# myrrix/myrrix-recommender

Measured on AMD Instinct MI355X. Metric: ALS rows solved/sec (full iteration) at k=64, higher is better.
Workload: dtype f32 storage; per-row Gramian: f16x2-split operands (22 bits), f32 accumulate; Cholesky f32

## Files before the change

### myrrix-recommender_amd/csrc/als_kernels.h

```cpp
#pragma once
#include <hip/hip_runtime.h>
#include <stdint.h>

#include <type_traits>

#include "work_plan.h"

namespace mals {

#ifndef MALS_WAVES
#define MALS_WAVES(T, MODE) ((T) <= 4 ? 4 : ((T) == 5 ? 3 : 2))
#endif
#ifndef MALS_WAVES_H
#define MALS_WAVES_H(T, MODE) ((T) <= 2 ? 5 : ((T) <= 4 ? 3 : 2))
#endif

typedef float f32x4 __attribute__((ext_vector_type(4)));
typedef double f64x4 __attribute__((ext_vector_type(4)));

__host__ __device__ constexpr int tri(int T) { return T * (T + 1) / 2; }
__host__ __device__ constexpr int tidx(int T, int i, int j) { return i * T - (i * (i - 1)) / 2 + (j - i); }

constexpr int GRAMIAN_FLUSH_BINADES = 5;
constexpr int YMAX_SLOTS = 64;
// ... 557 lines not shown
    }
    pp.ch = chn;
  }
}

typedef _Float16 f16x8 __attribute__((ext_vector_type(8)));
typedef _Float16 f16x4 __attribute__((ext_vector_type(4)));
typedef _Float16 f16x2 __attribute__((ext_vector_type(2)));
typedef int i32x4 __attribute__((ext_vector_type(4)));
typedef int i32x2 __attribute__((ext_vector_type(2)));

template <int E>
struct ZOp {
  int r[E / 2];
};
template <int E>
__device__ __forceinline__ f32x4 mfma_h(const ZOp<E>& a, const ZOp<E>& b, f32x4 c) {
  if constexpr (E == 8) {
    return __builtin_amdgcn_mfma_f32_16x16x32_f16(__builtin_bit_cast(f16x8, a), __builtin_bit_cast(f16x8, b), c, 0, 0, 0);
  } else {
    return __builtin_amdgcn_mfma_f32_16x16x16f16(__builtin_bit_cast(f16x4, a), __builtin_bit_cast(f16x4, b), c, 0, 0, 0);
  }
}
#ifndef MALS_SPLIT8_MAXT
#define MALS_SPLIT8_MAXT 7
#endif
__host__ __device__ constexpr int split_slots(int T) { return T <= MALS_SPLIT8_MAXT ? 8 : 4; }

__device__ __forceinline__ void chunk_weights_h(const SolveParams& p, Chunk& e, float zscale) {
  chunk_weights(p, e);
  e.w = __builtin_amdgcn_sqrtf(e.w) * zscale;
}

template <int T, int E, bool FULL, int E2>
__device__ __forceinline__ void issue_pair_h(const SolveParams& p, int col_src, int off, int lane, float (&raw)[T][E]) {
  const int c = lane & 15;
  int col[2];
  bperm2_i<8 * E2, 8 * E2 + 4>(off, col_src, col[0], col[1]);
#ifdef MALS_PROFILING
  if (p.flags & 0x400) {
    col[0] &= 0xfff;
    col[1] &= 0xfff;
  }
#endif
#pragma unroll
  for (int i = 0; i < 2; ++i) {
    const int e = 2 * E2 + i;
    const float* ptr = p.M + ((uint64_t)(uint32_t)col[i] * (uint32_t)p.ldm + (uint32_t)c);
#pragma unroll
    for (int v = 0; v < T; ++v) raw[v][e] = ptr[16 * v];
  }
}

template <int E2>
__device__ __forceinline__ void fetch_pair_cols_h(int col_src, int off, int (&col)[2]) {
  bperm2_i_start<8 * E2, 8 * E2 + 4>(off, col_src, col[0], col[1]);
}
template <int T, int E, bool FULL, int E2>
__device__ __forceinline__ void issue_pair_loads_h(const SolveParams& p, int (&col)[2], int lane, float (&raw)[T][E]) {
  const int c = lane & 15;
  bperm2_i_land(col[0], col[1]);
#ifdef MALS_PROFILING
  if (p.flags & 0x400) {
    col[0] &= 0xfff;
    col[1] &= 0xfff;
  }
#endif
#pragma unroll
  for (int i = 0; i < 2; ++i) {
    const int e = 2 * E2 + i;
    const float* ptr = p.M + ((uint64_t)(uint32_t)col[i] * (uint32_t)p.ldm + (uint32_t)c);
#pragma unroll
    for (int v = 0; v < T; ++v) raw[v][e] = ptr[16 * v];
  }
}

template <int T, int E, bool FULL, int PART, int E2, int NTERM = 2>
__device__ __forceinline__ void convert_pair_h(const SolveParams& p, const Chunk& ch, int lane, const float (&raw)[T][E], ZOp<E> (&zh)[T],
                                               ZOp<E> (&zl)[T], float (&bpart)[T], ZOp<E> (&zm)[NTERM == 3 ? T : 1]) {
  constexpr int m0 = E * PART + 2 * E2;
  const float s0 = row_bcast<m0>(ch.w), s1 = row_bcast<m0 + 1>(ch.w);
  const float c0 = row_bcast<m0>(ch.cb), c1 = row_bcast<m0 + 1>(ch.cb);
#pragma unroll
  for (int v = 0; v < T; ++v) {
    const float y0 = raw[v][2 * E2], y1 = raw[v][2 * E2 + 1];
    const float z0 = y0 * s0, z1 = y1 * s1;
    const int hp = pk_rn16(z0, z1);
    const f16x2 hh = __builtin_bit_cast(f16x2, hp);
    zh[v].r[E2] = hp;
    if constexpr (NTERM == 3) {
      const float r0 = fmaf((float)hh[0], -1.f, z0), r1 = fmaf((float)hh[1], -1.f, z1);
      const int mp = pk_rn16(r0, r1);
      const f16x2 mh = __builtin_bit_cast(f16x2, mp);
      zm[v].r[E2] = mp;
      zl[v].r[E2] = pk_rn16(fmaf((float)mh[0], -1.f, r0), fmaf((float)mh[1], -1.f, r1));
    } else {
      zl[v].r[E2] = pk_rn16(fmaf((float)hh[0], -1.f, z0), fmaf((float)hh[1], -1.f, z1));
    }
    bpart[v] = fmaf(c0, y0, bpart[v]);
    bpart[v] = fmaf(c1, y1, bpart[v]);
  }
}

template <int T, int E, bool FULL, int PART, int NTERM = 2>
__device__ __forceinline__ void convert_refill_h(const SolveParams& p, const Chunk& ch, int next_col, int next_off, int lane,
                                                 float (&raw)[T][E], ZOp<E> (&zh)[T], ZOp<E> (&zl)[T], float (&bpart)[T], ZOp<E> (&zm)[NTERM == 3 ? T : 1]) {
#define MALS_SB __builtin_amdgcn_sched_barrier(0)
  int col[2];
  fetch_pair_cols_h<0>(next_col, next_off, col);
  MALS_SB;
  convert_pair_h<T, E, FULL, PART, 0, NTERM>(p, ch, lane, raw, zh, zl, bpart, zm);
  MALS_SB;
  issue_pair_loads_h<T, E, FULL, 0>(p, col, lane, raw);
  fetch_pair_cols_h<1>(next_col, next_off, col);
  MALS_SB;
  convert_pair_h<T, E, FULL, PART, 1, NTERM>(p, ch, lane, raw, zh, zl, bpart, zm);
  MALS_SB;
  issue_pair_loads_h<T, E, FULL, 1>(p, col, lane, raw);
  if constexpr (E == 8) {
    fetch_pair_cols_h<2>(next_col, next_off, col);
    MALS_SB;
    convert_pair_h<T, E, FULL, PART, 2, NTERM>(p, ch, lane, raw, zh, zl, bpart, zm);
    MALS_SB;
    issue_pair_loads_h<T, E, FULL, 2>(p, col, lane, raw);
    fetch_pair_cols_h<3>(next_col, next_off, col);
    MALS_SB;
    convert_pair_h<T, E, FULL, PART, 3, NTERM>(p, ch, lane, raw, zh, zl, bpart, zm);
    MALS_SB;
    issue_pair_loads_h<T, E, FULL, 3>(p, col, lane, raw);
  }
#undef MALS_SB
}

template <int T, int E>
__device__ __forceinline__ void gram_super_step(const ZOp<E> (&zh)[T], const ZOp<E> (&zl)[T], f32x4 (&acc)[tri(T)]) {
#pragma unroll
  for (int i = 0; i < T; ++i)
#pragma unroll
    for (int j = i; j < T; ++j) acc[tidx(T, i, j)] = mfma_h<E>(zh[i], zh[j], acc[tidx(T, i, j)]);
#pragma unroll
  for (int i = 0; i < T; ++i)
#pragma unroll
    for (int j = i; j < T; ++j) acc[tidx(T, i, j)] = mfma_h<E>(zh[i], zl[j], acc[tidx(T, i, j)]);
#pragma unroll
  for (int i = 0; i < T; ++i)
#pragma unroll
    for (int j = i; j < T; ++j) acc[tidx(T, i, j)] = mfma_h<E>(zl[i], zh[j], acc[tidx(T, i, j)]);
}

template <int T, int E>
__device__ __forceinline__ void gram_super_step3(const ZOp<E> (&zh)[T], const ZOp<E> (&zm)[T], const ZOp<E> (&zl)[T], f32x4 (&acc)[tri(T)]) {
#define MALS_GS3(A, B)                                                                                    \
  _Pragma("unroll") for (int i = 0; i < T; ++i) _Pragma("unroll") for (int j = i; j < T; ++j)              \
      acc[tidx(T, i, j)] = mfma_h<E>(A[i], B[j], acc[tidx(T, i, j)])
  MALS_GS3(zl, zh);
  MALS_GS3(zh, zl);
  MALS_GS3(zm, zm);
  MALS_GS3(zm, zh);
  MALS_GS3(zh, zm);
  MALS_GS3(zh, zh);
#undef MALS_GS3
}

template <int T, int E, bool FULL>
__device__ __forceinline__ void prime_row_h(const SolveParams& p, int col_src, int lane, float (&raw)[T][E]) {
  const int rb = (lane & 48) << 2;
  issue_pair_h<T, E, FULL, 0>(p, col_src, rb, lane, raw);
  issue_pair_h<T, E, FULL, 1>(p, col_src, rb, lane, raw);
  if constexpr (E == 8) {
    issue_pair_h<T, E, FULL, 2>(p, col_src, rb, lane, raw);
    issue_pair_h<T, E, FULL, 3>(p, col_src, rb, lane, raw);
  }
}

template <int T, int E, bool FULL, int PART, int NTERM = 2>
__device__ __forceinline__ void super_step_h(const SolveParams& p, const Chunk& ch, const Chunk& chn, int next_col, bool last, int lane,
                                             float (&raw)[T][E], f32x4 (&acc)[tri(T)], float (&bpart)[T]) {
  constexpr int NP = 16 / E;
  const int rb = (lane & 48) << 2;
  ZOp<E> zh[T], zl[T], zm[NTERM == 3 ? T : 1];
  const int same_row_col = PART == NP - 1 ? chn.col : ch.col;
  const int same_row_off = PART == NP - 1 ? rb : rb + 4 * E * (PART + 1);
  convert_refill_h<T, E, FULL, PART, NTERM>(p, ch, last ? next_col : same_row_col, last ? rb : same_row_off, lane, raw, zh, zl, bpart, zm);
  __builtin_amdgcn_sched_barrier(0);
  if constexpr (NTERM == 3) gram_super_step3<T, E>(zh, zm, zl, acc);
  else gram_super_step<T, E>(zh, zl, acc);
  __builtin_amdgcn_sched_barrier(0);
}

template <int T, int E, bool FULL, int NTERM = 2>
__device__ __forceinline__ void gather_row_h(const SolveParams& p, int64_t begin, int len, int lane, float zscale, Chunk& ch,
                                             int next_col, float (&raw)[T][E], f32x4 (&acc)[tri(T)], float (&bpart)[T]) {
  constexpr int NS = 4 * E, NP = 16 / E;
  const int n_ss = (len + NS - 1) / NS;
  for (int q = 0; NP * q < n_ss; ++q) {
    Chunk chn = chunk_issue<true>(p, begin, len, 64 * (q + 1), lane);
    const int ss = NP * q;
    super_step_h<T, E, FULL, 0, NTERM>(p, ch, chn, next_col, ss + 1 >= n_ss, lane, raw, acc, bpart);
    if (ss + 1 < n_ss) {
      if (NP == 2) chunk_weights_h(p, chn, zscale);
      super_step_h<T, E, FULL, 1, NTERM>(p, ch, chn, next_col, ss + 2 >= n_ss, lane, raw, acc, bpart);
    }
    if constexpr (NP == 4) {
      if (ss + 2 < n_ss) super_step_h<T, E, FULL, 2, NTERM>(p, ch, chn, next_col, ss + 3 >= n_ss, lane, raw, acc, bpart);
      if (ss + 3 < n_ss) {
        chunk_weights_h(p, chn, zscale);
        super_step_h<T, E, FULL, 3, NTERM>(p, ch, chn, next_col, ss + 4 >= n_ss, lane, raw, acc, bpart);
      }
    }
    ch = chn;
  }
}

template <int T>
__device__ __forceinline__ void init_acc(const SolveParams& p, f32x4 (&acc)[tri(T)], int lane) {
  if (!(p.flags & 2)) {
    const f32x4* G4 = reinterpret_cast<const f32x4*>(p.Gf) + lane;
#pragma unroll
    for (int t = 0; t < tri(T); ++t) acc[t] = G4[t * 64];
  } else {
#pragma unroll
    for (int t = 0; t < tri(T); ++t) acc[t] = f32x4{0.f, 0.f, 0.f, 0.f};
  }
}

template <int T, bool FULL = false>
__device__ __forceinline__ void add_ridge(const SolveParams& p, f32x4 (&acc)[tri(T)], int n_u, int lane) {
  const int g = lane >> 4, c = lane & 15;
  const float ridge = p.lambda_alpha * (float)n_u;
  float rd[4];
#pragma unroll
  for (int r = 0; r < 4; ++r) rd[r] = (4 * g + r == c) ? ridge : 0.f;
  float w00 = 1.f;
  if constexpr (!FULL) w00 = readlane(acc[tidx(T, 0, 0)][0], 0) + ridge;
#pragma unroll
  for (int v = 0; v < T; ++v) {
    if (FULL || v < T - 1) {
#pragma unroll
      for (int r = 0; r < 4; ++r) acc[tidx(T, v, v)][r] += rd[r];
    } else {
// ... 56 lines not shown
    } else {
#pragma unroll
      for (int r = 0; r < 4; ++r) acc[t][r] *= s2;
    }
  }
#pragma unroll
  for (int v = 0; v < T; ++v) bcol[v] *= s2;
  return inv_s2;
}

template <int T, bool PERM = false>
__device__ __forceinline__ void store_row(const SolveParams& p, float (&xcol)[T], float minpiv, float wmax, int row, int lane) {
  if (!(minpiv > p.sing_threshold)) {
    if (lane == 0) {
      if (p.refine_flag) {
        p.refine_flag[row] = 2;
        *p.any_marked = 1;
      } else {
        atomicMin(p.bad_row, (unsigned long long)row);
      }
    }
#pragma unroll
    for (int v = 0; v < T; ++v) xcol[v] = 0.f;
  } else {
    if (minpiv <= 1024.f * p.sing_threshold && lane == 0) {
      const unsigned long long key = ((unsigned long long)__float_as_uint(minpiv) << 32) | (unsigned)row;
      if (key < __builtin_nontemporal_load(p.suspect)) atomicMin(p.suspect, key);
    }
    if (p.refine_flag && p.refine_limit > 0.f && wmax > p.refine_limit * minpiv && lane == 0) {
      p.refine_flag[row] = 1;
      *p.any_marked = 1;
    }
  }
  if constexpr (PERM) {
    static_assert(T == 8, "the permuted feature order belongs to the k = 128 kernels");
    float* o = p.out + (int64_t)row * p.k;
    int l2 = lane;
    asm volatile("" : "+v"(l2));
    const int g = l2 >> 4, c = l2 & 15;
    const bool hi = ((g ^ (c >> 3)) & 1) != 0;
    f32x4 x;
#pragma unroll
    for (int q = 0; q < 4; ++q) x[q] = hi ? xcol[4 + q] : xcol[q];
    if (g < 2) *reinterpret_cast<f32x4*>(o + 8 * c + 4 * g) = x;
  } else {
    float* o = p.out + (int64_t)row * p.k;
    int l2 = lane;
    asm volatile("" : "+v"(l2));
    const int g = l2 >> 4, c = l2 & 15;
#pragma unroll
    for (int m = 0; 4 * m < T; ++m) {
      const float x = select4(g, xcol[4 * m], 4 * m + 1 < T ? xcol[4 * m + 1] : 0.f, 4 * m + 2 < T ? xcol[4 * m + 2] : 0.f,
                              4 * m + 3 < T ? xcol[4 * m + 3] : 0.f);
      const int feat = 16 * (4 * m + g) + c;
      if (4 * m + 3 < T - 1 || feat < p.k) o[feat] = x;
    }
  }
}

template <int T, bool PERM = false>
__device__ __forceinline__ void finish_row(const SolveParams& p, f32x4 (&acc)[tri(T)], const float (&bcol)[T],
                                           int n_u, int row, int lane, float rmax = 0.f) {
  add_ridge<T, PERM>(p, acc, n_u, lane);
  float minpiv = 3.0e38f;
  float xcol[T];
  const float wmax = fmaxf(rmax, p.gramian_weight * __int_as_float(max_entry_bits<T>(acc, lane)));
  cholesky_tiles<T>(acc, lane, minpiv);
  solve_tiles<T>(acc, bcol, xcol, lane);
// ... 94 lines not shown
          chunk_weights(p, pp.ch);
          prime_row<T, D, FULL>(p, lane, pp);
        }
        solve_tiles<T>(acc, bcol, xcol, lane);
      }
      store_row<T>(p, xcol, minpiv, wmax, cur.id, lane);
#ifdef MALS_PROFILING
      if (tr) {
        t3 = __builtin_readcyclecounter();
        if (lane == 0) {
          unsigned long long* o = p.trace + (trow * 64 + wave) * 6;
          o[0] = t0; o[1] = t1; o[2] = t2; o[3] = t3; o[4] = (unsigned long long)cur.len; o[5] = wall_clock64();
        }
      }
#endif
    } else {
      float* s = p.scratch + (int64_t)cur.id * ((tri(T) * 4 + T) * 64);
#pragma unroll
      for (int t = 0; t < tri(T); ++t) reinterpret_cast<f32x4*>(s)[t * 64 + lane] = acc[t];
#pragma unroll
      for (int v = 0; v < T; ++v) s[(tri(T) * 4 + v) * 64 + lane] = bcol[v];
      if (prime_next) {
        chunk_weights(p, pp.ch);
        prime_row<T, D, FULL>(p, lane, pp);
      }
    }
    if (nxt.len < 0) break;
    cur = nxt;
    nxt = nxt2;
    it += n_waves;
  }
}

template <int T, int MODE, bool FULL, int NTERM = 2>
__global__ __launch_bounds__(256, MALS_WAVES_H(T, MODE)) void als_persistent_kernel_h(SolveParams p) {
  __shared__ f32x4 sG[MODE == 0 ? tri(T) * 64 : 1];
  const int lane = threadIdx.x & 63;
  const int wave = uniform(blockIdx.x * 4 + (threadIdx.x >> 6));
  const int64_t n_waves = (int64_t)gridDim.x * 4;
  if (MODE == 0) {
    const f32x4* G4 = reinterpret_cast<const f32x4*>(p.Gf);
    for (int e = threadIdx.x; e < tri(T) * 64; e += 256) sG[e] = (p.flags & 2) ? f32x4{0.f, 0.f, 0.f, 0.f} : G4[e];
    __syncthreads();
  }
  int64_t it = wave;
  if (it >= p.n_work) return;
  if (p.zscale[2] == 0.f) return;
  const float zscale = __int_as_float(uniform(__float_as_int(p.zscale[0])));
  const float inv_s2 = __int_as_float(uniform(__float_as_int(p.zscale[1])));
  WorkItem cur = load_item(p, it);
  WorkItem nxt = load_item(p, it + n_waves);
  WorkItem nx2 = load_item(p, it + 2 * n_waves);
  constexpr int E = split_slots(T);
  float raw[T][E];
#pragma unroll
  for (int v = 0; v < T; ++v)
#pragma unroll
    for (int e = 0; e < E; ++e) raw[v][e] = 0.f;
  if (cur.len > 0) {
    Chunk ch = chunk_issue<true>(p, cur.begin, cur.len, 0, lane);
    Chunk nch = nxt.len > 0 ? chunk_issue<true>(p, nxt.begin, nxt.len, 0, lane) : ch;
    chunk_weights_h(p, ch, zscale);
    prime_row_h<T, E, FULL>(p, ch.col, lane, raw);
    for (;;) {
      const WorkItem nx3 = load_item(p, it + 3 * n_waves);
      f32x4 acc[tri(T)];
#pragma unroll
      for (int t = 0; t < tri(T); ++t) acc[t] = f32x4{0.f, 0.f, 0.f, 0.f};
      float bpart[T];
#pragma unroll
      for (int v = 0; v < T; ++v) bpart[v] = 0.f;
#ifdef MALS_PROFILING
      const int64_t trow = it / n_waves - p.trace_start;
      const bool tr = MODE == 0 && p.trace && wave < 64 && trow >= 0 && trow < 64;
      unsigned long long t0 = 0, t1 = 0, t2 = 0;
      if (tr) t0 = __builtin_readcyclecounter();
#endif
      gather_row_h<T, E, FULL, NTERM>(p, cur.begin, cur.len, lane, zscale, ch, nch.col, raw, acc, bpart);
#ifdef MALS_PROFILING
      if (tr) t1 = __builtin_readcyclecounter();
#endif
      float bcol[T];
#pragma unroll
      for (int v = 0; v < T; ++v) bcol[v] = reduce_groups(bpart[v], lane);
      ch = nch;
      if (nxt.len > 0) chunk_weights_h(p, ch, zscale);
      if (MODE == 0) {
        const float rmax = p.refine_flag ? __int_as_float(max_entry_bits<T>(acc, lane)) * inv_s2 : 0.f;
#pragma unroll
        for (int t = 0; t < tri(T); ++t) {
          const f32x4 g4 = sG[t * 64 + lane];
          if constexpr (T <= MALS_PK_MAXT) {
            acc[t] = __builtin_elementwise_fma(acc[t], f32x4{inv_s2, inv_s2, inv_s2, inv_s2}, g4);
          } else {
#pragma unroll
            for (int r = 0; r < 4; ++r) acc[t][r] = fmaf(acc[t][r], inv_s2, g4[r]);
          }
        }
        add_ridge<T, FULL>(p, acc, cur.len, lane);
        float minpiv = 3.0e38f, wmax;
        float xcol[T];
        if constexpr (T >= 2) {
          const float inv_s2row = row_scale<T>(acc, bcol, lane, wmax);
          cholesky_tiles<T, true>(acc, lane, minpiv);
          minpiv *= inv_s2row;
        } else {
          wmax = __int_as_float(max_entry_bits<T>(acc, lane));
          cholesky_tiles<T>(acc, lane, minpiv);
        }
#ifdef MALS_PROFILING
        if (tr) t2 = __builtin_readcyclecounter();
#endif
        solve_tiles<T>(acc, bcol, xcol, lane);
        store_row<T>(p, xcol, minpiv, fmaxf(rmax, p.gramian_weight * wmax), cur.id, lane);
#ifdef MALS_PROFILING
        if (tr) {
          const unsigned long long t3 = __builtin_readcyclecounter();
          if (lane == 0) {
            unsigned long long* o = p.trace + (trow * 64 + wave) * 6;
            o[0] = t0; o[1] = t1; o[2] = t2; o[3] = t3; o[4] = (unsigned long long)cur.len; o[5] = wall_clock64();
          }
        }
#endif
      } else {
        float* s = p.scratch + (int64_t)cur.id * ((tri(T) * 4 + T) * 64);
#pragma unroll
        for (int t = 0; t < tri(T); ++t) reinterpret_cast<f32x4*>(s)[t * 64 + lane] = acc[t] * inv_s2;
#pragma unroll
        for (int v = 0; v < T; ++v) s[(tri(T) * 4 + v) * 64 + lane] = bcol[v];
      }
      cur = nxt;
      nxt = nx2;
      nx2 = nx3;
      nch = nxt.len > 0 ? chunk_issue<true>(p, nxt.begin, nxt.len, 0, lane) : nch;
      it += n_waves;
      if (cur.len <= 0) break;
    }
  }
  if (MODE == 0) {
    while (cur.len == 0) {
      f32x4 acc[tri(T)];
#pragma unroll
      for (int t = 0; t < tri(T); ++t) acc[t] = sG[t * 64 + lane];
      float bcol[T];
#pragma unroll
      for (int v = 0; v < T; ++v) bcol[v] = 0.f;
      finish_row<T>(p, acc, bcol, 0, cur.id, lane);
      it += n_waves;
      cur = load_item(p, it);
    }
  }
}

template <int T>
__device__ __forceinline__ void add_slot(const float* __restrict__ s, int lane, f32x4 (&acc)[tri(T)], float (&bcol)[T]) {
  constexpr int PASSES = T >= 6 ? 2 : 1, PER = (tri(T) + PASSES - 1) / PASSES;
#pragma unroll
  for (int ps = 0; ps < PASSES; ++ps) {
    f32x4 part[PER];
#pragma unroll
    for (int t = 0; t < PER; ++t)
      if (ps * PER + t < tri(T)) part[t] = reinterpret_cast<const f32x4*>(s)[(ps * PER + t) * 64 + lane];
    if (ps == 0) {
      float bp[T];
#pragma unroll
      for (int v = 0; v < T; ++v) bp[v] = s[(tri(T) * 4 + v) * 64 + lane];
#pragma unroll
      for (int v = 0; v < T; ++v) bcol[v] += bp[v];
    }
#pragma unroll
    for (int t = 0; t < PER; ++t)
      if (ps * PER + t < tri(T)) acc[ps * PER + t] += part[t];
    if (PASSES > 1) __builtin_amdgcn_sched_barrier(0);
  }
}

template <int T>
__global__ __launch_bounds__(256) void als_prereduce_kernel(SolveParams p) {
  const int lane = threadIdx.x & 63;
  const int64_t wave = (int64_t)blockIdx.x * 4 + (threadIdx.x >> 6);
// ... 824 lines not shown
```

### myrrix-recommender_amd/csrc/lds_kernels.h

```cpp
#pragma once
#include "als_kernels.h"

namespace mals {

constexpr int LDSK_T = 8, LDSK_E = 8;
#ifndef MALS_LDSK_RESPLIT
#define MALS_LDSK_RESPLIT 1
#endif
constexpr bool LDSK_RESPLIT = MALS_LDSK_RESPLIT != 0;
constexpr int LDSK_ROW_BYTES = 512;
constexpr int LDSK_RING_BYTES = 32 * LDSK_ROW_BYTES;
constexpr int LDSK_CHUNK_BYTES = 512;
constexpr int LDSK_NCHUNK = 3;
constexpr int LDSK_WAVE_BYTES = LDSK_RING_BYTES + LDSK_NCHUNK * LDSK_CHUNK_BYTES;

__host__ __device__ constexpr int ldsk_feature(int v, int c) { return 8 * c + (v ^ (4 * (c >> 3))); }

typedef __attribute__((address_space(3))) char lds_char;

__device__ __forceinline__ void glds16(const void* a, unsigned dst) {
  unsigned keep;
  asm volatile(
      "s_mov_b32 %0, m0\n\t"
      "s_mov_b32 m0, %2\n\ts_nop 0\n\tglobal_load_lds_dwordx4 %1, off\n\t"
// ... 77 lines not shown

template <int E2>
__device__ __forceinline__ void ldsk_pair(const lds_char* lds, unsigned ring, float w, float cb, unsigned next_cols, const LdskLane& L,
                                          ZOp<LDSK_E> (&zh)[LDSK_T], ZOp<LDSK_E> (&zl)[LDSK_T], float (&bpart)[LDSK_T]) {
  wait_vm<12>();
  const float s0 = row_bcast<2 * E2>(w), s1 = row_bcast<2 * E2 + 1>(w);
  const float c0 = row_bcast<2 * E2>(cb), c1 = row_bcast<2 * E2 + 1>(cb);
  {
    const f32x4 ya = *reinterpret_cast<lds_f4>(lds + L.rd0 + 4096 * E2);
    const f32x4 yb = *reinterpret_cast<lds_f4>(lds + L.rd0 + 4096 * E2 + 512);
    ldsk_convert_half<E2, 0>(ya, yb, s0, s1, c0, c1, zh, zl, bpart);
  }
  __builtin_amdgcn_sched_barrier(0);
  {
    const f32x4 ya = *reinterpret_cast<lds_f4>(lds + (L.rd0 ^ 16u) + 4096 * E2);
    const f32x4 yb = *reinterpret_cast<lds_f4>(lds + (L.rd0 ^ 16u) + 4096 * E2 + 512);
    ldsk_convert_half<E2, 4>(ya, yb, s0, s1, c0, c1, zh, zl, bpart);
  }
  __builtin_amdgcn_sched_barrier(0);
  ldsk_issue_pair<E2>(lds, ring, next_cols, L);
  __builtin_amdgcn_sched_barrier(0);
}
__device__ __forceinline__ void ldsk_super_step(const lds_char* lds, unsigned ring, float w, float cb, unsigned next_cols, const LdskLane& L,
                                                f32x4 (&acc)[tri(LDSK_T)], float (&bpart)[LDSK_T]) {
  ZOp<LDSK_E> zh[LDSK_T], zl[LDSK_T];
  ldsk_pair<0>(lds, ring, w, cb, next_cols, L, zh, zl, bpart);
  ldsk_pair<1>(lds, ring, w, cb, next_cols, L, zh, zl, bpart);
  ldsk_pair<2>(lds, ring, w, cb, next_cols, L, zh, zl, bpart);
  ldsk_pair<3>(lds, ring, w, cb, next_cols, L, zh, zl, bpart);
  gram_super_step<LDSK_T, LDSK_E>(zh, zl, acc);
  __builtin_amdgcn_sched_barrier(0);
}

__global__ void gramian_perm_kernel(const double* __restrict__ G, int k, float* __restrict__ Gp) {
  constexpr int T = LDSK_T;
  const int e = blockIdx.x * blockDim.x + threadIdx.x;
  if (e >= tri(T) * 256) return;
  const int t = e >> 8, lane = (e >> 2) & 63, reg = e & 3;
  int i = 0, rem = t;
  while (rem >= T - i) {
    rem -= T - i;
    ++i;
  }
  const int j = i + rem;
  const int row = ldsk_feature(i, 4 * (lane >> 4) + reg), col = ldsk_feature(j, lane & 15);
  Gp[e] = (row < k && col < k) ? (float)G[(int64_t)row * k + col] : 0.f;
}

template <int MODE>
__global__ __launch_bounds__(64, 2) void als_lds_kernel_h(SolveParams p) {
  constexpr int T = LDSK_T;
  __shared__ __attribute__((aligned(1024))) char lds_raw[LDSK_WAVE_BYTES];
  const lds_char* lds = (const lds_char*)lds_raw;
  const unsigned lbase = (unsigned)(uintptr_t)lds;
  const int lane = threadIdx.x;
  const int64_t wave = blockIdx.x, n_waves = gridDim.x;
  int64_t it = wave;
  if (it >= p.n_work) return;
  if (p.zscale[2] == 0.f) return;
  const float zscale = __int_as_float(uniform(__float_as_int(p.zscale[0])));
  const float inv_s2 = __int_as_float(uniform(__float_as_int(p.zscale[1])));
  LdskLane L;
  {
    const int g = lane >> 4, c = lane & 15;
    L.rd0 = (unsigned)(g * 1024 + 32 * c + 16 * (c >> 3));
    L.gsrc = reinterpret_cast<const char*>(p.M) + 16 * (lane & 31);
  }
  const unsigned ring = lbase;
  unsigned b_cur = LDSK_RING_BYTES, b_next = LDSK_RING_BYTES + LDSK_CHUNK_BYTES, b_nrow = LDSK_RING_BYTES + 2 * LDSK_CHUNK_BYTES;
  const f32x4* Gp4 = reinterpret_cast<const f32x4*>(p.Gperm);
  WorkItem cur = load_item(p, it);
  WorkItem nxt = load_item(p, it + n_waves);
  WorkItem nx2 = load_item(p, it + 2 * n_waves);
  if (cur.len > 0) {
    ldsk_chunk_dma(p, cur.begin, cur.len, 0, lbase + b_cur, lane);
    if (nxt.len > 0) ldsk_chunk_dma(p, nxt.begin, nxt.len, 0, lbase + b_nrow, lane);
    wait_vm<0>();
    {
// ... 121 lines not shown
```

### myrrix-recommender_amd/csrc/mals_api.hip

```cpp
#include "../../include/myrrix_als.h"
#include "als_kernels.h"
#include "dual_kernels.h"
#include "lds_kernels.h"
#include "host_eigen.h"
#include "host_solver.h"
#include "mals_internal.h"
#include "mals_handle.h"
#include "hip_buffer.h"
#include "work_plan.h"

#include <hip/hip_runtime.h>

#include <algorithm>
#include <chrono>
#include <cmath>
#include <cstdio>
#include <cstdlib>
#include <cstring>
#include <limits>
#include <new>
#include <string>
#include <type_traits>
#include <vector>

// ... 372 lines not shown
    if (!r.n) continue;
    p.n_work = r.n;
    p.items = r.items;
    if (int rc = r.kind ? launch_persistent(h, fam.segments, fam.segments_f32, fam.block, fam.resident_per_cu, p, 1, r.bytes, r.front)
                        : launch_persistent(h, fam.rows, fam.rows_f32, fam.block, fam.resident_per_cu, p, 0, r.bytes, r.front))
      return rc;
  }
  if (longs && cr.nC) {
    PendingEvent pe;
    if (int rc = begin_timed(h, 2, (double)cr.nC * per, pe)) return rc;
    if (cr.nP) {
      p.n_work = cr.nP;
      p.rowsC = s.rowsC.get() + cr.offP;
      hipLaunchKernelGGL(fam.prereduce, dim3((unsigned)((cr.nP + 3) / 4)), dim3(256), 0, h->stream, p);
    }
    p.n_work = cr.nC;
    p.rowsC = s.rowsC.get() + cr.offC;
    hipLaunchKernelGGL(fam.finish, dim3((unsigned)((cr.nC + 3) / 4)), dim3(256), 0, h->stream, p);
    if constexpr (!std::is_same<decltype(fam.finish_f32), std::nullptr_t>::value) {
      SolveParams pf = p;
      pf.flags |= 8;
      hipLaunchKernelGGL(fam.finish_f32, dim3((unsigned)((cr.nC + 3) / 4)), dim3(256), 0, h->stream, pf);
    }
    if (int rc = end_timed(h, pe)) return rc;
  }
  if (own && cr.nZ) {
    hipLaunchKernelGGL(zero_rows_kernel, dim3((unsigned)((cr.nZ + 31) / 32)), dim3(256), 0, h->stream,
                       A + cr.nA + n_dual, cr.nZ, p.k, p.out);
  }
  HIPCHK(h, hipGetLastError());
  return MALS_OK;
}

template <int T, bool FULL>
int launch_solve_TF(mals_handle h, SideState& s, const SolveParams& p, int chunk, int which) {
  constexpr int D = gather_depth(T);
  constexpr auto rows_f32 = als_persistent_kernel<T, D, 0, FULL>;
  constexpr auto segments_f32 = als_persistent_kernel<T, D, 1, FULL>;
  if constexpr (T == 8 && FULL) {
    if (h->split_f16 && h->lds_gather && p.Gperm)
      return launch_lists(h, s, p, chunk, which, ListKernels{als_lds_kernel_h<0>, als_lds_kernel_h<1>, rows_f32, segments_f32, als_finish_kernel<T, true>,
                                                             als_finish_kernel<T, false>, als_prereduce_kernel<T>, 64, 8});
  }
  if constexpr (T == 4) {
    if (h->split3)
      return launch_lists(h, s, p, chunk, which, ListKernels{als_persistent_kernel_h<T, 0, FULL, 3>, als_persistent_kernel_h<T, 1, FULL, 3>, rows_f32,
                                                             segments_f32, als_finish_kernel<T>, nullptr, als_prereduce_kernel<T>, 256, 0});
  }
  if (h->split_f16)
    return launch_lists(h, s, p, chunk, which, ListKernels{als_persistent_kernel_h<T, 0, FULL>, als_persistent_kernel_h<T, 1, FULL>, rows_f32,
                                                           segments_f32, als_finish_kernel<T>, nullptr, als_prereduce_kernel<T>, 256, 0});
  return launch_lists(h, s, p, chunk, which,
                      ListKernels{rows_f32, segments_f32, nullptr, nullptr, als_finish_kernel<T>, nullptr, als_prereduce_kernel<T>, 256, 0});
}

int launch_solve(mals_handle h, SideState& s, const SolveParams& p, int chunk, int which) {
  return dispatch_T(h, [&](auto t) {
    return p.k == 16 * t() ? launch_solve_TF<t(), true>(h, s, p, chunk, which) : launch_solve_TF<t(), false>(h, s, p, chunk, which);
  });
}

int launch_refine(mals_handle h, const RefineParams& q) {
  const int64_t rows = q.row_end - q.row_begin;
  const unsigned grid = (unsigned)std::max<int64_t>(1, std::min<int64_t>((rows + 255) / 256, (int64_t)h->n_cu * 8));
  return dispatch_T(h, [&](auto t) -> int {
    hipLaunchKernelGGL((als_refine_kernel<t()>), dim3(grid), dim3(256), 0, h->stream, q);
    HIPCHK(h, hipGetLastError());
    return MALS_OK;
  });
}

int launch_gramian_ref(mals_handle h, const SideState& o) {
  const unsigned grid = (unsigned)std::max<int64_t>(1, std::min<int64_t>((o.n_total + 63) / 64, (int64_t)h->n_cu * 2));
  return dispatch_T(h, [&](auto t) -> int {
    hipLaunchKernelGGL(gramian_ref_latch_kernel, dim3(1), dim3(1), 0, h->stream, h->d_gref_state.get());
// ... 425 lines not shown
  }
  if (h->cfg.flags != 0 || !(cfg->alpha > 0.0)) h->dual_blocks = 0;
  {
    hipDeviceProp_t prop;
    if (hipGetDeviceProperties(&prop, cfg->device) == hipSuccess && prop.multiProcessorCount > 0)
      h->n_cu = prop.multiProcessorCount;
  }
  std::memset(&h->stats, 0, sizeof(h->stats));
  h->stats.struct_size = (int32_t)sizeof(mals_stats);
  hipError_t st = hipSetDevice(cfg->device);
  if (st == hipSuccess) st = h->d_bad.alloc(4);
  if (st == hipSuccess) st = h->h_bad.alloc(4);
  if (st == hipSuccess) st = h->d_zscale.alloc(4);
  if (st == hipSuccess) st = h->d_maxabs.alloc(4);
  if (st == hipSuccess) st = h->d_colrange.alloc(2);
  if (st == hipSuccess) st = h->d_refined.alloc(1);
  if (st == hipSuccess) st = h->d_gref_state.alloc(4);
  if (st == hipSuccess) st = hipMemset(h->d_gref_state.get(), 0, 4 * sizeof(int));
  if (st == hipSuccess) st = hipMemset(h->d_refined.get(), 0, sizeof(unsigned long long));
  if (st == hipSuccess) st = hipMemset(h->d_zscale.get(), 0, 4 * sizeof(float));
  if (st == hipSuccess) st = hipMemset(h->d_bad.get(), 0xff, 4 * sizeof(unsigned long long));
  if (st != hipSuccess) {
    delete h;
    return create_fail(MALS_HIP_ERROR, "mals_create: device " + std::to_string(cfg->device) + ": " + hipGetErrorString(st));
  }
  if (const char* e = std::getenv("MALS_REFINE_LIMIT")) h->refine_limit = std::max(0.f, (float)std::atof(e));
  if (hipEventCreateWithFlags(&h->ev_ready, hipEventDisableTiming) != hipSuccess ||
      hipEventCreateWithFlags(&h->ev_refine, hipEventDisableTiming) != hipSuccess) {
    delete h;
    return create_fail(MALS_HIP_ERROR, "mals_create: hipEventCreate failed");
  }
  h->lds_gather = h->cfg.features == 128;
  if (const char* e = std::getenv("MALS_LDS_GATHER")) h->lds_gather = h->lds_gather && std::atoi(e) != 0;
  if (const char* e = std::getenv("MALS_OVERLAP")) h->overlap = std::atoi(e) != 0;
  if (h->overlap) {
    bool ok = hipEventCreateWithFlags(&h->ev_fork, hipEventDisableTiming) == hipSuccess;
    for (int i = 0; i < 2 && ok; ++i)
      ok = hipStreamCreateWithFlags(&h->aux[i], hipStreamNonBlocking) == hipSuccess &&
           hipEventCreateWithFlags(&h->ev_join[i], hipEventDisableTiming) == hipSuccess;
    if (!ok) h->overlap = false;
  }
#ifdef MALS_PROFILING
  if (std::getenv("MALS_DEBUG_TRACE")) {
    (void)h->d_trace.alloc(64 * 64 * 6);
    (void)hipMemset(h->d_trace.get(), 0, 64 * 64 * 6 * sizeof(unsigned long long));
  }
#endif
  t_create_error.clear();
  malsi_serving_create(h);
  *out = h;
  return MALS_OK;
}

int mals_destroy(mals_handle h) {
  if (!h) return MALS_INVALID_ARG;
  (void)hipSetDevice(h->cfg.device);
  malsi_serving_stop_front(h);
  (void)hipStreamSynchronize(h->stream);
  if (h->d_trace) {
    std::vector<unsigned long long> t(64 * 64 * 6);
    (void)hipMemcpy(t.data(), h->d_trace.get(), t.size() * sizeof(unsigned long long), hipMemcpyDeviceToHost);
    for (int r = 0; r < 64; r += 21)
      for (int w = 0; w < 4; w += 1) {
        const unsigned long long* o = &t[(size_t)(r * 64 + w) * 6];
        std::fprintf(stderr, "[trace] iter %2d wave %2d len %5llu gather %7llu chol %7llu solve+store %7llu gap_to_prev_end %lld\n", r, w, o[4],
                     o[1] - o[0], o[2] - o[1], o[3] - o[2], r ? (long long)(o[0] - t[(size_t)((r - 1) * 64 + w) * 6 + 3]) : 0ll);
// ... 398 lines not shown
static int solve_setup(mals_handle h, int side, int chunk_begin, int chunk_end, bool g_to_host) {
  SideState& s = h->side[side];
  SideState& o = h->side[1 - side];
  const int k = h->cfg.features;
  const HalfStamp now{side, o.G_version};
  bool new_half = h->pad != now || h->pad_epoch != o.F_epoch || h->pad_done.size() != s.chunks.size();
  for (int c = chunk_begin; c < chunk_end && !new_half; ++c) new_half = h->pad_done[(size_t)c] != 0;
  if (new_half) {
    h->pad = now;
    h->pad_epoch = o.F_epoch;
    h->pad_done.assign(s.chunks.size(), 0);
    h->tl[0] = now_us();
    h->tl[1] = h->tl[2] = 0.0;
    HIPCHK(h, hipMemsetAsync(h->d_gref_state.get(), 0, 3 * sizeof(int), h->stream));
  }
  for (int c = chunk_begin; c < chunk_end; ++c) h->pad_done[(size_t)c] = 1;
  if (k % 16 != 0) {
    const int ld = 16 * h->T;
    const size_t need = (size_t)o.n_total * (size_t)ld;
    if (need > h->d_Mp.capacity()) {
      new_half = true;
      HIPCHK(h, h->d_Mp.reserve(need, h->stream));
    }
    if (new_half) {
      PendingEvent pe;
      if (int rc = begin_timed(h, 5, (double)o.n_total * 4.0 * (k + ld), pe)) return rc;
      const int64_t n4 = o.n_total * (ld / 4);
      const unsigned blocks = (unsigned)std::min<int64_t>((n4 + 255) / 256, (int64_t)h->n_cu * 32);
      hipLaunchKernelGGL(pad_rows_kernel, dim3(blocks ? blocks : 1), dim3(256), 0, h->stream, o.F, o.n_total, k, ld, h->d_Mp.get());
      HIPCHK(h, hipGetLastError());
      if (int rc = end_timed(h, pe)) return rc;
    }
  }
  if (h->lds_gather && h->split_f16 && k == 128) {
    if (!h->d_Gperm) HIPCHK(h, h->d_Gperm.alloc((size_t)tri(8) * 256));
    if (h->gperm != now) {
      if (h->cfg.flags & MALS_FLAG_LOSS_IGNORES_UNSPECIFIED) {
        HIPCHK(h, hipMemsetAsync(h->d_Gperm.get(), 0, sizeof(float) * (size_t)tri(8) * 256, h->stream));
      } else {
        hipLaunchKernelGGL(gramian_perm_kernel, dim3((unsigned)tri(8)), dim3(256), 0, h->stream, o.G.get(), k, h->d_Gperm.get());
        HIPCHK(h, hipGetLastError());
      }
      h->gperm = now;
    }
  }
  HIPCHK(h, s.refine.reserve((size_t)s.n_local, h->stream));
  if (h->split_f16 && (h->zs != now || h->zs_bound != s.max_abs_val || h->zs_mean != s.mean_abs_val)) {
    const double base_w = (h->cfg.flags & MALS_FLAG_LOSS_IGNORES_UNSPECIFIED) ? 1.0 : 0.0;
    const double w_max = base_w + ((h->cfg.flags & MALS_FLAG_RECONSTRUCT_R) ? 0.0 : std::fabs(h->cfg.alpha) * (double)s.max_abs_val);
    const double w_mean = base_w + ((h->cfg.flags & MALS_FLAG_RECONSTRUCT_R) ? 0.0 : std::fabs(h->cfg.alpha) * s.mean_abs_val);
    int force = -1;
    if (const char* e = std::getenv("MALS_FORCE_RANGE_FLAG")) force = std::atoi(e) != 0;
    hipLaunchKernelGGL(gather_scale_kernel, dim3(1), dim3(64), 0, h->stream, o.G.get(), k, (float)std::sqrt(w_max), (float)std::sqrt(w_mean),
                       (double)o.n_total, force, (o.ymax_version != 0 && o.ymax_version == o.G_version) ? o.d_ymax.get() : nullptr, h->d_zscale.get());
    HIPCHK(h, hipGetLastError());
    h->zs = now;
    h->zs_bound = s.max_abs_val;
    h->zs_mean = s.mean_abs_val;
  }
  if (g_to_host) {
    if (!h->h_G) HIPCHK(h, h->h_G.alloc((size_t)k * k));
    if (!h->ev_G) HIPCHK(h, hipEventCreateWithFlags(&h->ev_G, hipEventDisableTiming));
    HIPCHK(h, hipMemcpyAsync(h->h_G.get(), o.G.get(), sizeof(double) * (size_t)k * k, hipMemcpyDeviceToHost, h->stream));
    HIPCHK(h, hipEventRecord(h->ev_G, h->stream));
  }
  return MALS_OK;
}

static SolveParams solve_params(mals_handle h, int side) {
  SideState& s = h->side[side];
  SideState& o = h->side[1 - side];
  const int k = h->cfg.features;
  SolveParams p;
  p.row_ptr = s.row_ptr;
  p.col = s.col;
  p.val = s.val;
  p.M = o.F;
  p.ldm = k;
  if (k % 16 != 0) {
    p.M = h->d_Mp.get();
    p.ldm = 16 * h->T;
  }
  p.Gf = o.Gf.get();
  p.Gperm = h->lds_gather && h->split_f16 && k == 128 ? h->d_Gperm.get() : nullptr;
  p.out = s.F + s.row_offset * k;
  p.items = nullptr;
  p.rowsC = s.rowsC.get();
  p.scratch = s.scratch.get();
  p.bad_row = h->d_bad.get() + side;
  p.suspect = h->d_bad.get() + 2 + side;
  p.any_marked = h->d_gref_state.get();
  p.refine_flag = s.refine.get();
  p.refine_limit = (h->cfg.flags & MALS_FLAG_LOSS_IGNORES_UNSPECIFIED) ? h->refine_limit / 16.f : h->refine_limit;
  p.gramian_weight = 0.25f;
  if (h->cfg.flags & MALS_FLAG_RECONSTRUCT_R) {
    p.gramian_weight = 1.f;
    p.refine_limit *= 0.25f;
  }
  p.n_work = 0;
  p.trace = h->d_trace.get();
  p.trace_start = 0;
  if (const char* ts = std::getenv("MALS_DEBUG_TRACE")) p.trace_start = std::atoi(ts);
  if (const char* ts = std::getenv("MALS_DEBUG_TRACE_SIDE")) if (std::atoi(ts) != side) p.trace = nullptr;
  p.k = k;
  p.flags = h->cfg.flags;
  p.alpha = (float)h->cfg.alpha;
  p.lambda_alpha = (float)(h->cfg.lambda * h->cfg.alpha);
  p.sing_threshold = (float)h->cfg.singularity_threshold;
  p.zscale = h->d_zscale.get();
  return p;
}

static int solve_one_chunk(mals_handle h, int side, const SolveParams& p, int c, int phase, bool want_dual, bool prepare_dual, bool* dual_now) {
  SideState& s = h->side[side];
  const SideState& o = h->side[1 - side];
  const ChunkRange& cr = s.chunks[(size_t)c];
  const bool resume = phase == SOLVE_END;
// ... 520 lines not shown
```

### myrrix-recommender_amd/csrc/mals_handle.h

```cpp
#pragma once
#include "../../include/myrrix_als.h"
#include "hip_buffer.h"
#include "host_solver.h"
#include "work_plan.h"

#include <hip/hip_runtime.h>

#include <atomic>
#include <cstdint>
#include <string>
#include <vector>

struct ServingState;

namespace mals __attribute__((visibility("hidden"))) {

struct SideState {
  int64_t n_total = 0;
  float* F = nullptr;
  DeviceBuffer<float> F_own;
  int64_t row_offset = 0, n_local = 0, nnz = 0;
  int64_t* row_ptr = nullptr;
  int32_t* col = nullptr;
  float* val = nullptr;
// ... 73 lines not shown
  float refine_limit = 64.f;
  bool exact_ready = false;
  DeviceBuffer<int> d_gref_state;
  DeviceBuffer<double> d_Gref;
  DeviceBuffer<double> d_gref_part;
  DeviceBuffer<unsigned long long> d_refined;
  HalfStamp pad;
  uint64_t pad_epoch = 0;
  std::vector<uint8_t> pad_done;
  DeviceBuffer<char> d_eig;
  double* d_Q = nullptr;
  float* d_Qf = nullptr;
  bool rotate_f64 = false;
  bool rotate_split = false;
  int32_t* d_Bs = nullptr;
  size_t Bs_stride = 0;
  float* d_lam = nullptr;
  DeviceBuffer<unsigned> d_zbound;
  PinnedBuffer<double> h_G;
  hipEvent_t ev_G = nullptr;
  PinnedBuffer<char> eig_stage;
  bool eig_ok = false;
  double eig_gmax = 0.0;
  bool dual_pending = false;
  int dual_pending_side = -1, dual_pending_chunk = -1;
  double tl[4] = {0.0, 0.0, 0.0, 0.0};
  HalfStamp dual;
  bool dual_ok = false;
  hipEvent_t ev_ready = nullptr, ev_refine = nullptr;
  bool refine_recorded = false;
  mals_iteration_fn iter_fn = nullptr;
  void* iter_user = nullptr;
  bool lds_gather = false;
  DeviceBuffer<float> d_Gperm;
  HalfStamp gperm;
  DeviceBuffer<float> d_zscale;
  HalfStamp zs;
  float zs_bound = -1.f;
  double zs_mean = -1.0;
  DeviceBuffer<unsigned> d_maxabs;
  DeviceBuffer<int> d_colrange;
  int n_cu = 256;
  SideState side[2];
  hipStream_t stream = nullptr;
  hipStream_t aux[2] = {nullptr, nullptr};
  hipEvent_t ev_fork = nullptr, ev_join[2] = {nullptr, nullptr};
  bool overlap = false;
  bool forked[2] = {false, false};
  std::string err;
  DeviceBuffer<unsigned long long> d_bad;
  PinnedBuffer<unsigned long long> h_bad;
  int32_t sing_side = -1;
  int64_t sing_row = -1;
  int32_t sing_rank = 0;
  std::atomic<int> cancelled{0};
  bool timing = false;
  mals_stats stats;
  std::vector<PendingEvent> pending;
  DeviceBuffer<unsigned long long> d_trace;
  ServingState* serving = nullptr;
  DeviceBuffer<uint32_t> tag_bits;
  int64_t tag_bits_items = 0, n_tag_items = 0;
  const int64_t* known_ptr = nullptr;
  const int32_t* known_idx = nullptr;
  int64_t known_rows = 0;
  DeviceBuffer<int64_t> known_ptr_copy;
// ... 75 lines not shown
```

Before: 139.0 million.

## Use permuted feature order for k=64 so each lane gathers one 16-byte vector

For k=64 row solves, lane c now owns features 4c..4c+3, so each gathered factor row entry is fetched with a single 16-byte vector load instead of four strided scalar loads. The prior Gramian is permuted to match on the device, and the solved row is written back with a 16-byte store from 16 lanes. This cuts gather instruction count and should improve coalescing on the memory-bound gather. The cost is an extra Gperm buffer and permute kernel whenever the Gramian changes, plus more kernel instantiations.

```diff
diff --git a/myrrix-recommender_amd/csrc/als_kernels.h b/myrrix-recommender_amd/csrc/als_kernels.h
--- a/myrrix-recommender_amd/csrc/als_kernels.h
+++ b/myrrix-recommender_amd/csrc/als_kernels.h
@@ -613,7 +613,27 @@
   e.w = __builtin_amdgcn_sqrtf(e.w) * zscale;
 }
 
-template <int T, int E, bool FULL, int E2>
+__host__ __device__ constexpr int perm4_feature(int v, int c) { return 4 * c + v; }
+template <int T, int E, bool FULL, bool PERM>
+__device__ __forceinline__ void load_entry_h(const SolveParams& p, int col, int c, int e, float (&raw)[T][E]) {
+#ifdef MALS_GATHER16_ABLATION
+  constexpr bool X4 = T == 4 && E == 8 && FULL;
+#else
+  constexpr bool X4 = PERM;
+#endif
+  if constexpr (X4) {
+    static_assert(T == 4 && FULL, "the 16-byte gather belongs to k = 64");
+    const f32x4 q = *reinterpret_cast<const f32x4*>(p.M + ((uint64_t)(uint32_t)col * (uint32_t)p.ldm + (uint32_t)(4 * c)));
+#pragma unroll
+    for (int v = 0; v < T; ++v) raw[v][e] = q[v];
+  } else {
+    const float* ptr = p.M + ((uint64_t)(uint32_t)col * (uint32_t)p.ldm + (uint32_t)c);
+#pragma unroll
+    for (int v = 0; v < T; ++v) raw[v][e] = ptr[16 * v];
+  }
+}
+
+template <int T, int E, bool FULL, int E2, bool PERM = false>
 __device__ __forceinline__ void issue_pair_h(const SolveParams& p, int col_src, int off, int lane, float (&raw)[T][E]) {
   const int c = lane & 15;
   int col[2];
@@ -627,9 +647,7 @@
 #pragma unroll
   for (int i = 0; i < 2; ++i) {
     const int e = 2 * E2 + i;
-    const float* ptr = p.M + ((uint64_t)(uint32_t)col[i] * (uint32_t)p.ldm + (uint32_t)c);
-#pragma unroll
-    for (int v = 0; v < T; ++v) raw[v][e] = ptr[16 * v];
+    load_entry_h<T, E, FULL, PERM>(p, col[i], c, e, raw);
   }
 }
 
@@ -637,7 +655,7 @@
 __device__ __forceinline__ void fetch_pair_cols_h(int col_src, int off, int (&col)[2]) {
   bperm2_i_start<8 * E2, 8 * E2 + 4>(off, col_src, col[0], col[1]);
 }
-template <int T, int E, bool FULL, int E2>
+template <int T, int E, bool FULL, int E2, bool PERM = false>
 __device__ __forceinline__ void issue_pair_loads_h(const SolveParams& p, int (&col)[2], int lane, float (&raw)[T][E]) {
   const int c = lane & 15;
   bperm2_i_land(col[0], col[1]);
@@ -650,9 +668,7 @@
 #pragma unroll
   for (int i = 0; i < 2; ++i) {
     const int e = 2 * E2 + i;
-    const float* ptr = p.M + ((uint64_t)(uint32_t)col[i] * (uint32_t)p.ldm + (uint32_t)c);
-#pragma unroll
-    for (int v = 0; v < T; ++v) raw[v][e] = ptr[16 * v];
+    load_entry_h<T, E, FULL, PERM>(p, col[i], c, e, raw);
   }
 }
 
@@ -683,7 +699,7 @@
   }
 }
 
-template <int T, int E, bool FULL, int PART, int NTERM = 2>
+template <int T, int E, bool FULL, int PART, int NTERM = 2, bool PERM = false>
 __device__ __forceinline__ void convert_refill_h(const SolveParams& p, const Chunk& ch, int next_col, int next_off, int lane,
                                                  float (&raw)[T][E], ZOp<E> (&zh)[T], ZOp<E> (&zl)[T], float (&bpart)[T], ZOp<E> (&zm)[NTERM == 3 ? T : 1]) {
 #define MALS_SB __builtin_amdgcn_sched_barrier(0)
@@ -692,23 +708,23 @@
   MALS_SB;
   convert_pair_h<T, E, FULL, PART, 0, NTERM>(p, ch, lane, raw, zh, zl, bpart, zm);
   MALS_SB;
-  issue_pair_loads_h<T, E, FULL, 0>(p, col, lane, raw);
+  issue_pair_loads_h<T, E, FULL, 0, PERM>(p, col, lane, raw);
   fetch_pair_cols_h<1>(next_col, next_off, col);
   MALS_SB;
   convert_pair_h<T, E, FULL, PART, 1, NTERM>(p, ch, lane, raw, zh, zl, bpart, zm);
   MALS_SB;
-  issue_pair_loads_h<T, E, FULL, 1>(p, col, lane, raw);
+  issue_pair_loads_h<T, E, FULL, 1, PERM>(p, col, lane, raw);
   if constexpr (E == 8) {
     fetch_pair_cols_h<2>(next_col, next_off, col);
     MALS_SB;
     convert_pair_h<T, E, FULL, PART, 2, NTERM>(p, ch, lane, raw, zh, zl, bpart, zm);
     MALS_SB;
-    issue_pair_loads_h<T, E, FULL, 2>(p, col, lane, raw);
+    issue_pair_loads_h<T, E, FULL, 2, PERM>(p, col, lane, raw);
     fetch_pair_cols_h<3>(next_col, next_off, col);
     MALS_SB;
     convert_pair_h<T, E, FULL, PART, 3, NTERM>(p, ch, lane, raw, zh, zl, bpart, zm);
     MALS_SB;
-    issue_pair_loads_h<T, E, FULL, 3>(p, col, lane, raw);
+    issue_pair_loads_h<T, E, FULL, 3, PERM>(p, col, lane, raw);
   }
 #undef MALS_SB
 }
@@ -743,18 +759,18 @@
 #undef MALS_GS3
 }
 
-template <int T, int E, bool FULL>
+template <int T, int E, bool FULL, bool PERM = false>
 __device__ __forceinline__ void prime_row_h(const SolveParams& p, int col_src, int lane, float (&raw)[T][E]) {
   const int rb = (lane & 48) << 2;
-  issue_pair_h<T, E, FULL, 0>(p, col_src, rb, lane, raw);
-  issue_pair_h<T, E, FULL, 1>(p, col_src, rb, lane, raw);
+  issue_pair_h<T, E, FULL, 0, PERM>(p, col_src, rb, lane, raw);
+  issue_pair_h<T, E, FULL, 1, PERM>(p, col_src, rb, lane, raw);
   if constexpr (E == 8) {
-    issue_pair_h<T, E, FULL, 2>(p, col_src, rb, lane, raw);
-    issue_pair_h<T, E, FULL, 3>(p, col_src, rb, lane, raw);
-  }
-}
-
-template <int T, int E, bool FULL, int PART, int NTERM = 2>
+    issue_pair_h<T, E, FULL, 2, PERM>(p, col_src, rb, lane, raw);
+    issue_pair_h<T, E, FULL, 3, PERM>(p, col_src, rb, lane, raw);
+  }
+}
+
+template <int T, int E, bool FULL, int PART, int NTERM = 2, bool PERM = false>
 __device__ __forceinline__ void super_step_h(const SolveParams& p, const Chunk& ch, const Chunk& chn, int next_col, bool last, int lane,
                                              float (&raw)[T][E], f32x4 (&acc)[tri(T)], float (&bpart)[T]) {
   constexpr int NP = 16 / E;
@@ -762,14 +778,14 @@
   ZOp<E> zh[T], zl[T], zm[NTERM == 3 ? T : 1];
   const int same_row_col = PART == NP - 1 ? chn.col : ch.col;
   const int same_row_off = PART == NP - 1 ? rb : rb + 4 * E * (PART + 1);
-  convert_refill_h<T, E, FULL, PART, NTERM>(p, ch, last ? next_col : same_row_col, last ? rb : same_row_off, lane, raw, zh, zl, bpart, zm);
+  convert_refill_h<T, E, FULL, PART, NTERM, PERM>(p, ch, last ? next_col : same_row_col, last ? rb : same_row_off, lane, raw, zh, zl, bpart, zm);
   __builtin_amdgcn_sched_barrier(0);
   if constexpr (NTERM == 3) gram_super_step3<T, E>(zh, zm, zl, acc);
   else gram_super_step<T, E>(zh, zl, acc);
   __builtin_amdgcn_sched_barrier(0);
 }
 
-template <int T, int E, bool FULL, int NTERM = 2>
+template <int T, int E, bool FULL, int NTERM = 2, bool PERM = false>
 __device__ __forceinline__ void gather_row_h(const SolveParams& p, int64_t begin, int len, int lane, float zscale, Chunk& ch,
                                              int next_col, float (&raw)[T][E], f32x4 (&acc)[tri(T)], float (&bpart)[T]) {
   constexpr int NS = 4 * E, NP = 16 / E;
@@ -777,16 +793,16 @@
   for (int q = 0; NP * q < n_ss; ++q) {
     Chunk chn = chunk_issue<true>(p, begin, len, 64 * (q + 1), lane);
     const int ss = NP * q;
-    super_step_h<T, E, FULL, 0, NTERM>(p, ch, chn, next_col, ss + 1 >= n_ss, lane, raw, acc, bpart);
+    super_step_h<T, E, FULL, 0, NTERM, PERM>(p, ch, chn, next_col, ss + 1 >= n_ss, lane, raw, acc, bpart);
     if (ss + 1 < n_ss) {
       if (NP == 2) chunk_weights_h(p, chn, zscale);
-      super_step_h<T, E, FULL, 1, NTERM>(p, ch, chn, next_col, ss + 2 >= n_ss, lane, raw, acc, bpart);
+      super_step_h<T, E, FULL, 1, NTERM, PERM>(p, ch, chn, next_col, ss + 2 >= n_ss, lane, raw, acc, bpart);
     }
     if constexpr (NP == 4) {
-      if (ss + 2 < n_ss) super_step_h<T, E, FULL, 2, NTERM>(p, ch, chn, next_col, ss + 3 >= n_ss, lane, raw, acc, bpart);
+      if (ss + 2 < n_ss) super_step_h<T, E, FULL, 2, NTERM, PERM>(p, ch, chn, next_col, ss + 3 >= n_ss, lane, raw, acc, bpart);
       if (ss + 3 < n_ss) {
         chunk_weights_h(p, chn, zscale);
-        super_step_h<T, E, FULL, 3, NTERM>(p, ch, chn, next_col, ss + 4 >= n_ss, lane, raw, acc, bpart);
+        super_step_h<T, E, FULL, 3, NTERM, PERM>(p, ch, chn, next_col, ss + 4 >= n_ss, lane, raw, acc, bpart);
       }
     }
     ch = chn;
@@ -909,8 +925,13 @@
       *p.any_marked = 1;
     }
   }
-  if constexpr (PERM) {
-    static_assert(T == 8, "the permuted feature order belongs to the k = 128 kernels");
+  if constexpr (PERM && T == 4) {
+    float* o = p.out + (int64_t)row * p.k;
+    int l2 = lane;
+    asm volatile("" : "+v"(l2));
+    if (l2 < 16) *reinterpret_cast<f32x4*>(o + 4 * l2) = f32x4{xcol[0], xcol[1], xcol[2], xcol[3]};
+  } else if constexpr (PERM) {
+    static_assert(T == 8, "the permuted feature orders belong to the k = 64 and k = 128 kernels");
     float* o = p.out + (int64_t)row * p.k;
     int l2 = lane;
     asm volatile("" : "+v"(l2));
@@ -1071,14 +1092,15 @@
   }
 }
 
-template <int T, int MODE, bool FULL, int NTERM = 2>
+template <int T, int MODE, bool FULL, int NTERM = 2, bool PERM = false>
 __global__ __launch_bounds__(256, MALS_WAVES_H(T, MODE)) void als_persistent_kernel_h(SolveParams p) {
+  static_assert(!PERM || (T == 4 && FULL && MODE == 0), "the permuted feature order is the k = 64 rows kernel's");
   __shared__ f32x4 sG[MODE == 0 ? tri(T) * 64 : 1];
   const int lane = threadIdx.x & 63;
   const int wave = uniform(blockIdx.x * 4 + (threadIdx.x >> 6));
   const int64_t n_waves = (int64_t)gridDim.x * 4;
   if (MODE == 0) {
-    const f32x4* G4 = reinterpret_cast<const f32x4*>(p.Gf);
+    const f32x4* G4 = reinterpret_cast<const f32x4*>(PERM ? p.Gperm : p.Gf);
     for (int e = threadIdx.x; e < tri(T) * 64; e += 256) sG[e] = (p.flags & 2) ? f32x4{0.f, 0.f, 0.f, 0.f} : G4[e];
     __syncthreads();
   }
@@ -1100,7 +1122,7 @@
     Chunk ch = chunk_issue<true>(p, cur.begin, cur.len, 0, lane);
     Chunk nch = nxt.len > 0 ? chunk_issue<true>(p, nxt.begin, nxt.len, 0, lane) : ch;
     chunk_weights_h(p, ch, zscale);
-    prime_row_h<T, E, FULL>(p, ch.col, lane, raw);
+    prime_row_h<T, E, FULL, PERM>(p, ch.col, lane, raw);
     for (;;) {
       const WorkItem nx3 = load_item(p, it + 3 * n_waves);
       f32x4 acc[tri(T)];
@@ -1115,7 +1137,7 @@
       unsigned long long t0 = 0, t1 = 0, t2 = 0;
       if (tr) t0 = __builtin_readcyclecounter();
 #endif
-      gather_row_h<T, E, FULL, NTERM>(p, cur.begin, cur.len, lane, zscale, ch, nch.col, raw, acc, bpart);
+      gather_row_h<T, E, FULL, NTERM, PERM>(p, cur.begin, cur.len, lane, zscale, ch, nch.col, raw, acc, bpart);
 #ifdef MALS_PROFILING
       if (tr) t1 = __builtin_readcyclecounter();
 #endif
@@ -1151,7 +1173,7 @@
         if (tr) t2 = __builtin_readcyclecounter();
 #endif
         solve_tiles<T>(acc, bcol, xcol, lane);
-        store_row<T>(p, xcol, minpiv, fmaxf(rmax, p.gramian_weight * wmax), cur.id, lane);
+        store_row<T, PERM>(p, xcol, minpiv, fmaxf(rmax, p.gramian_weight * wmax), cur.id, lane);
 #ifdef MALS_PROFILING
         if (tr) {
           const unsigned long long t3 = __builtin_readcyclecounter();
@@ -1184,7 +1206,7 @@
       float bcol[T];
 #pragma unroll
       for (int v = 0; v < T; ++v) bcol[v] = 0.f;
-      finish_row<T>(p, acc, bcol, 0, cur.id, lane);
+      finish_row<T, PERM>(p, acc, bcol, 0, cur.id, lane);
       it += n_waves;
       cur = load_item(p, it);
     }
diff --git a/myrrix-recommender_amd/csrc/lds_kernels.h b/myrrix-recommender_amd/csrc/lds_kernels.h
--- a/myrrix-recommender_amd/csrc/lds_kernels.h
+++ b/myrrix-recommender_amd/csrc/lds_kernels.h
@@ -133,8 +133,7 @@
   __builtin_amdgcn_sched_barrier(0);
 }
 
-__global__ void gramian_perm_kernel(const double* __restrict__ G, int k, float* __restrict__ Gp) {
-  constexpr int T = LDSK_T;
+__global__ void gramian_perm_kernel(const double* __restrict__ G, int k, int T, float* __restrict__ Gp) {
   const int e = blockIdx.x * blockDim.x + threadIdx.x;
   if (e >= tri(T) * 256) return;
   const int t = e >> 8, lane = (e >> 2) & 63, reg = e & 3;
@@ -144,7 +143,8 @@
     ++i;
   }
   const int j = i + rem;
-  const int row = ldsk_feature(i, 4 * (lane >> 4) + reg), col = ldsk_feature(j, lane & 15);
+  const int rc = 4 * (lane >> 4) + reg, cc = lane & 15;
+  const int row = T == LDSK_T ? ldsk_feature(i, rc) : perm4_feature(i, rc), col = T == LDSK_T ? ldsk_feature(j, cc) : perm4_feature(j, cc);
   Gp[e] = (row < k && col < k) ? (float)G[(int64_t)row * k + col] : 0.f;
 }
 
diff --git a/myrrix-recommender_amd/csrc/mals_api.hip b/myrrix-recommender_amd/csrc/mals_api.hip
--- a/myrrix-recommender_amd/csrc/mals_api.hip
+++ b/myrrix-recommender_amd/csrc/mals_api.hip
@@ -428,6 +428,10 @@
   return MALS_OK;
 }
 
+static bool uses_gperm(mals_handle h) {
+  return h->split_f16 && ((h->lds_gather && h->cfg.features == 128) || (h->gather16 && h->cfg.features == 64));
+}
+
 template <int T, bool FULL>
 int launch_solve_TF(mals_handle h, SideState& s, const SolveParams& p, int chunk, int which) {
   constexpr int D = gather_depth(T);
@@ -437,6 +441,15 @@
     if (h->split_f16 && h->lds_gather && p.Gperm)
       return launch_lists(h, s, p, chunk, which, ListKernels{als_lds_kernel_h<0>, als_lds_kernel_h<1>, rows_f32, segments_f32, als_finish_kernel<T, true>,
                                                              als_finish_kernel<T, false>, als_prereduce_kernel<T>, 64, 8});
+  }
+  if constexpr (T == 4 && FULL) {
+    if (h->split_f16 && h->gather16 && p.Gperm) {
+      if (h->split3)
+        return launch_lists(h, s, p, chunk, which, ListKernels{als_persistent_kernel_h<T, 0, FULL, 3, true>, als_persistent_kernel_h<T, 1, FULL, 3>, rows_f32,
+                                                               segments_f32, als_finish_kernel<T>, nullptr, als_prereduce_kernel<T>, 256, 0});
+      return launch_lists(h, s, p, chunk, which, ListKernels{als_persistent_kernel_h<T, 0, FULL, 2, true>, als_persistent_kernel_h<T, 1, FULL>, rows_f32,
+                                                             segments_f32, als_finish_kernel<T>, nullptr, als_prereduce_kernel<T>, 256, 0});
+    }
   }
   if constexpr (T == 4) {
     if (h->split3)
@@ -928,6 +941,8 @@
   }
   h->lds_gather = h->cfg.features == 128;
   if (const char* e = std::getenv("MALS_LDS_GATHER")) h->lds_gather = h->lds_gather && std::atoi(e) != 0;
+  h->gather16 = h->cfg.features == 64;
+  if (const char* e = std::getenv("MALS_K64_GATHER16")) h->gather16 = h->gather16 && std::atoi(e) != 0;
   if (const char* e = std::getenv("MALS_OVERLAP")) h->overlap = std::atoi(e) != 0;
   if (h->overlap) {
     bool ok = hipEventCreateWithFlags(&h->ev_fork, hipEventDisableTiming) == hipSuccess;
@@ -1392,13 +1407,13 @@
       if (int rc = end_timed(h, pe)) return rc;
     }
   }
-  if (h->lds_gather && h->split_f16 && k == 128) {
-    if (!h->d_Gperm) HIPCHK(h, h->d_Gperm.alloc((size_t)tri(8) * 256));
+  if (uses_gperm(h)) {
+    if (!h->d_Gperm) HIPCHK(h, h->d_Gperm.alloc((size_t)tri(h->T) * 256));
     if (h->gperm != now) {
       if (h->cfg.flags & MALS_FLAG_LOSS_IGNORES_UNSPECIFIED) {
-        HIPCHK(h, hipMemsetAsync(h->d_Gperm.get(), 0, sizeof(float) * (size_t)tri(8) * 256, h->stream));
+        HIPCHK(h, hipMemsetAsync(h->d_Gperm.get(), 0, sizeof(float) * (size_t)tri(h->T) * 256, h->stream));
       } else {
-        hipLaunchKernelGGL(gramian_perm_kernel, dim3((unsigned)tri(8)), dim3(256), 0, h->stream, o.G.get(), k, h->d_Gperm.get());
+        hipLaunchKernelGGL(gramian_perm_kernel, dim3((unsigned)tri(h->T)), dim3(256), 0, h->stream, o.G.get(), k, h->T, h->d_Gperm.get());
         HIPCHK(h, hipGetLastError());
       }
       h->gperm = now;
@@ -1442,7 +1457,7 @@
     p.ldm = 16 * h->T;
   }
   p.Gf = o.Gf.get();
-  p.Gperm = h->lds_gather && h->split_f16 && k == 128 ? h->d_Gperm.get() : nullptr;
+  p.Gperm = uses_gperm(h) ? h->d_Gperm.get() : nullptr;
   p.out = s.F + s.row_offset * k;
   p.items = nullptr;
   p.rowsC = s.rowsC.get();
diff --git a/myrrix-recommender_amd/csrc/mals_handle.h b/myrrix-recommender_amd/csrc/mals_handle.h
--- a/myrrix-recommender_amd/csrc/mals_handle.h
+++ b/myrrix-recommender_amd/csrc/mals_handle.h
@@ -129,6 +129,7 @@
   mals_iteration_fn iter_fn = nullptr;
   void* iter_user = nullptr;
   bool lds_gather = false;
+  bool gather16 = false;
   DeviceBuffer<float> d_Gperm;
   HalfStamp gperm;
   DeviceBuffer<float> d_zscale;
```

Result: no change. 140.3 million (median of 6 runs) (+0.9%).
